# nyenyu12/BioInformatics-project-for-Shotgun-Metagenomics-Pseudo-alignment-shotgun-

Hardware: AMD Instinct MI355X
Metric: reads/sec pseudo-aligned (k=31, 150bp) at 1/2/4/8 GPUs; % HBM roofline (higher is better)
Workload: dtype u8

## Files before the change

bioinformatics-project-for-shotgun-metagenomics-pseudo-alignment-shotgun-_amd/csrc/pa_align.hip:

```cpp
#include <hip/hip_runtime.h>

#include <algorithm>
#include <cstdio>
#include <cstdlib>
#include <cstring>
#include <vector>

#include "pa_device.h"
#include "pa_internal.h"

using namespace pad;

namespace {

constexpr int kBlock = 256;
constexpr int kWaves = kBlock / 64;
constexpr uint32_t kSegMaxWaves = 16384;
constexpr uint32_t kSegSlackWaves = 8192, kSegSlackChunks = 5;
constexpr uint64_t kSegSlack = 64ull * kSegSlackChunks * kSegSlackWaves;
constexpr uint32_t kLdsGenomeCap = 2048;

enum : uint32_t { F_MRQ = 1, F_MKQ = 2, F_MG = 4 };

struct AlignArgs {
// ... 626 lines not shown
                x.type_out[r] = type;
                x.qf_out[r] = qf;
                x.hr_out[r] = hr;
                x.len_out[r] = list_len;
            } else {
                atomicAdd(&a.stats[type == PA_UNMAPPED ? 2 : (type == PA_UNIQUELY_MAPPED ? 0 : 1)], 1ull);
                if (has_mkq && qf) atomicAdd(&a.stats[4], (unsigned long long)qf);
                if (has_mg && hr) atomicAdd(&a.stats[5], (unsigned long long)hr);
            }
        }
        __syncthreads();
    }
}


size_t fast_lds_bytes(uint32_t G, int wpl, bool need_q) {
    size_t cnt = G <= kLdsGenomeCap ? (((size_t)((G + 1) & ~1u) * 16 + 15) / 16 * 16) : 0;
    size_t wl = wpl == 1 ? fast_wave_bytes<1>(need_q) : wpl == 2 ? fast_wave_bytes<2>(need_q) : fast_wave_bytes<4>(need_q);
    return cnt + kWaves * wl;
}

template <int NW, int WPL, bool DENSE>
pa_status launch_fast(const AlignArgs &a, size_t shm, hipStream_t st) {
    auto kern = k_align_fast<NW, WPL, DENSE>;
    if (shm > 64 * 1024) PA_HIP(hipFuncSetAttribute((const void *)kern, hipFuncAttributeMaxDynamicSharedMemorySize, (int)shm));
    int per_cu = 0;
    PA_HIP(hipOccupancyMaxActiveBlocksPerMultiprocessor(&per_cu, kern, kBlock, shm));
    int dev = 0, cus = 256;
    PA_HIP(hipGetDevice(&dev));
    PA_HIP(hipDeviceGetAttribute(&cus, hipDeviceAttributeMultiprocessorCount, dev));
    uint64_t want = (a.n + kWaves - 1) / kWaves;
    uint64_t resident = (uint64_t)std::max(1, per_cu) * (uint64_t)cus;
    unsigned grid = (unsigned)std::max<uint64_t>(1, std::min<uint64_t>(want, resident));
    hipLaunchKernelGGL(kern, dim3(grid), dim3(kBlock), shm, st, a);
    PA_HIP(hipGetLastError());
    return PA_OK;
}

struct KernelTimer {
    pa_index *idx;
    hipStream_t st;
    int slot;
    hipEvent_t e0 = nullptr;
    KernelTimer(pa_index *i, hipStream_t s, int sl) : idx(i), st(s), slot(sl) {
        if (idx && idx->profile && hipEventCreate(&e0) == hipSuccess) hipEventRecord(e0, st);
    }
    ~KernelTimer() {
        hipEvent_t e1 = nullptr;
        if (e0 && hipEventCreate(&e1) == hipSuccess && hipEventRecord(e1, st) == hipSuccess)
            idx->kev.push_back({slot, e0, e1});
        else if (e0)
            hipEventDestroy(e0);
    }
};

constexpr uint64_t kRcnbMinReads = 32768;
pa_status launch_lane(const AlignArgs &a0, hipStream_t st, pa_index *prof = nullptr, bool long_reads = false,
                      int nw = 1) {
    const bool need_q = (a0.prm.flags & (F_MRQ | F_MKQ)) != 0;
    const bool win_q = (a0.prm.flags & F_MKQ) != 0;
    const bool mg = (a0.prm.flags & F_MG) != 0;
    const bool nm4 = long_reads && !win_q && nw == 1;
    AlignArgs a = a0;
    const size_t shm = lane_lds_bytes(a.G, nm4 ? 4 : 2, lane_sched(win_q, mg, nm4 ? 4 : 2, nw));
    auto kern = nw == 3
                    ? (win_q ? (mg ? k_align_lane<true, true, true, 2, 3> : k_align_lane<true, true, false, 2, 3>)
// ... 321 lines not shown

pa_status effective_params(const pa_reads *r, const DevParams &p, DevParams &out, hipStream_t st) {
    out = p;
    if (!(p.flags & (F_MRQ | F_MKQ)) || !r->qual || r->n == 0 || std::getenv("PA_NO_QELIDE")) return PA_OK;
    if (r->q_min < 0) PA_TRY(reads_measure(const_cast<pa_reads *>(r), st));
    if ((p.flags & F_MRQ) && r->len_min > 0 && p.mrq <= r->q_min) out.flags &= ~F_MRQ;
    if ((p.flags & F_MKQ) && p.mkq <= r->q_min) out.flags &= ~F_MKQ;
    return PA_OK;
}

pa_status align(pa_index *idx, const pa_reads *r, const DevParams &p_in, uint64_t base, pa_result *acc,
                hipStream_t st) {
    if (r->n == 0) return PA_OK;
    if (r->n >= 0xFFFFFFFFull) {
        set_error("pa_align: a batch holds at most 2^32 - 2 reads (split it; read_index_base keeps the order)");
        return PA_EUNSUPPORTED;
    }
    PA_TRY(index_note_reads(idx, r->n, st));
    PA_TRY(reserve_queues(idx, r->n));
    DevParams p;
    PA_TRY(effective_params(r, p_in, p, st));
    AlignArgs a = make_args(idx, r, p, base);
    const uint32_t G = idx->n_genomes;
    a.stats = (unsigned long long *)acc->sum_block;
    a.uniq = (unsigned long long *)acc->sum_block + 6;
    a.amb = a.uniq + G;
    a.first = (unsigned long long *)acc->min_block;
    a.queue = idx->queue;
    a.qcount = (unsigned long long *)idx->counters;
    a.deferred_total = (unsigned long long *)idx->counters + 1;
    a.dbg = (unsigned long long *)idx->counters + 4;
    PA_HIP(hipMemsetAsync(idx->counters, 0, 8, st));
#ifdef PA_STATS
    PA_HIP(hipMemsetAsync(a.dbg, 0, 224, st));
#endif
    ExactArgs x{};
    unsigned egrid = 0;
    PA_TRY(prepare_exact(idx, r, x, egrid));
    x.a = a;
    x.detail = 0;
    const bool fast_ok = idx->k > 0 && idx->nw <= 4 && idx->n_kmers > 0;
    const char *no_lane = std::getenv("PA_NO_LANE");
    const bool lane_ok = fast_ok && idx->nw <= 3 && a.tile_n > 0 && a.tile_lw && !(no_lane && no_lane[0] == '1');
    if (fast_ok) {
        const uint32_t wmax = r->max_len >= idx->k ? (uint32_t)(r->max_len - idx->k + 1) : 0;
        const int wpl = wmax <= 64 ? 1 : wmax <= 128 ? 2 : 4;
        hipEvent_t e0 = nullptr, e1 = nullptr;
        if (idx->profile) {
            PA_HIP(hipEventCreate(&e0));
            PA_HIP(hipEventCreate(&e1));
            PA_HIP(hipEventRecord(e0, st));
        }
        if (lane_ok) {
            if ((a.prm.flags & F_MG) && a.prm.mg >= 2) {
                const uint64_t n_words = a.tile_n / 64 + 8;
                if (!idx->tile_big) PA_HIP(pa::dev_malloc(&idx->tile_big, n_words * 8));
                if (idx->tile_big_mg != a.prm.mg) {
                    hipLaunchKernelGGL(k_tile_big, dim3((unsigned)std::min<uint64_t>((n_words + 3) / 4, 1u << 20)),
                                       dim3(256), 0, st, idx->tile_cls, a.tile_n, a.G, idx->class_genomes,
                                       (int32_t)a.prm.mg, idx->tile_big, n_words);
                    PA_HIP(hipGetLastError());
                    idx->tile_big_mg = a.prm.mg;
                }
                a.tile_big = idx->tile_big;
                if (idx->tile_nb && idx->nb_spec && !idx->tile_nb1 && !std::getenv("PA_NO_NBBIG")) {
                    const uint64_t nw = 3 * a.tile_n;
                    if (!idx->tile_nbbig) {
// ... 74 lines not shown
            a.na_min = 32768;
            if (const char *e = std::getenv("PA_NA_MIN")) a.na_min = std::strtoull(e, nullptr, 10);
            a.lane_next = (uint32_t *)(idx->na_count + 3);
            if (na || PA_LANE_CLAIM) PA_HIP(hipMemsetAsync(idx->na_count, 0, 32, st));
            const bool long_reads = r->max_len > (uint32_t)kLaneMaxLen ||
                                    (r->max_len >= idx->k && r->max_len - idx->k + 1 > (uint32_t)kLaneMaxW);
            PA_TRY(launch_lane(a, st, idx, long_reads, idx->nw));
            a.rlist = idx->queue_hard;
            a.rlist_count = a.queue_hard_count;
        }
        {
            KernelTimer kt(idx, st, PA_PROF_WAVE);
            PA_TRY(idx->nw == 1   ? launch_fast_wpl<1>(a, wpl, st)
                   : idx->nw == 2 ? launch_fast_wpl<2>(a, wpl, st)
                   : idx->nw == 3 ? launch_fast_wpl<3>(a, wpl, st)
                                  : launch_fast_wpl<4>(a, wpl, st));
        }
        if (idx->profile) {
            PA_HIP(hipEventRecord(e1, st));
            idx->ev_start.push_back(e0);
            idx->ev_stop.push_back(e1);
        }
        x.a = a;
        x.use_queue = 1;
    } else {
        x.use_queue = 0;
    }
    {
        KernelTimer kt(idx, st, PA_PROF_EXACT);
        launch_exact_nw(idx->nw, x, egrid, st);
        PA_HIP(hipGetLastError());
    }
#ifdef PA_STATS
    unsigned long long d[32];
    PA_HIP(hipMemcpyAsync(d, idx->counters, 256, hipMemcpyDeviceToHost, st));
    PA_HIP(hipStreamSynchronize(st));
    fprintf(stderr, "[pa_stats] reads %llu lane-hard %llu exact %llu | wave kernel: windows %llu probed %llu walk %llu anchors %llu\n",
            (unsigned long long)r->n, d[3], d[0], d[4], d[5], d[6], d[7]);
    fprintf(stderr, "[pa_stats] lane hard reasons: long %llu mkq %llu bad %llu no-anchor %llu range %llu mismatches %llu rep %llu found %llu pending %llu\n",
            d[8], d[9], d[10], d[11], d[12], d[13], d[14], d[15], d[16]);
    fprintf(stderr, "[pa_stats] lane: cooperative probes %llu re-anchors %llu neighbour words %llu | pending: invalid %llu "
            "2+ mismatches %llu neighbour present %llu\n", d[18], d[19], d[20], d[21], d[22], d[23]);
    fprintf(stderr, "[pa_stats] lane found: shared-neighbour+specific %llu second-walk specific %llu probed-shared+specific %llu"
            " | unique by bound %llu, by off-walk counts %llu | probes past the Bloom filter %llu\n", d[24], d[25], d[26], d[27], d[28],
            d[29]);
    fprintf(stderr, "[pa_stats] lane seeds: anchor ranked among stretches %llu, second seed round %llu\n", d[30], d[31]);
#endif
    return PA_OK;
}

pa_status align_detail(pa_index *idx, const pa_reads *r, const DevParams &p, uint8_t *type, uint32_t *qf,
                       uint32_t *hr, uint64_t *list_off, uint32_t *lists, uint64_t list_cap, uint64_t *list_total,
                       hipStream_t st) {
    const uint64_t n = r->n;
    if (list_off) list_off[0] = 0;
    if (list_total) *list_total = 0;
    if (n == 0) return PA_OK;
    ExactArgs x{};
    unsigned egrid = 0;
    PA_TRY(prepare_exact(idx, r, x, egrid));
    x.a = make_args(idx, r, p, 0);
    x.use_queue = 0;
    uint8_t *d_type = nullptr;
    uint32_t *d_qf = nullptr, *d_hr = nullptr, *d_len = nullptr, *d_lists = nullptr;
    uint64_t *d_off = nullptr;
    PA_HIP(pa::dev_malloc(&d_type, n));
    PA_HIP(pa::dev_malloc(&d_qf, n * 4));
    PA_HIP(pa::dev_malloc(&d_hr, n * 4));
    PA_HIP(pa::dev_malloc(&d_len, n * 4));
    x.type_out = d_type;
    x.qf_out = d_qf;
    x.hr_out = d_hr;
    x.len_out = d_len;
    x.detail = 1;
    launch_exact_nw(idx->nw, x, egrid, st);
// ... 65 lines not shown
```

bioinformatics-project-for-shotgun-metagenomics-pseudo-alignment-shotgun-_amd/csrc/pa_fast.h:

```cpp

#ifndef PA_HS_PER_WPL
#define PA_HS_PER_WPL 128
#endif
template <int WPL>
struct FastCfg {
    static constexpr int HS = PA_HS_PER_WPL * WPL;
    static constexpr int E = HS / 64;
    static constexpr int LCAP = 64 * WPL + 64;
    static constexpr int NDW = (LCAP + 8 + 255) / 256;
    static constexpr int PW = NDW * 8 + 2;
    static constexpr int BW = NDW * 4 + 2;
};

template <int WPL>
struct __align__(16) WaveLds {
    using C = FastCfg<WPL>;
    uint64_t packed[C::PW];
    uint64_t diff[C::PW];
    uint64_t poison[C::BW];
    uint64_t hA_key[C::HS];
    uint32_t hA_v[C::HS];
    uint32_t hA_v2[C::HS];
    uint32_t hB_key[C::HS];
    uint32_t hB_cnt[C::HS];
    uint32_t hB_min[C::HS];
    uint32_t gcnt[64];
    uint32_t gmin[64];
};

template <int WPL>
struct __align__(16) WaveQual {
    using C = FastCfg<WPL>;
    uint32_t stage[C::NDW * 64];
// ... 193 lines not shown
        }
#pragma unroll
        for (int e = 0; e < C::E; e++)
            if (bit(specm, e)) count_genome(a, wc, L.hB_key[lane + 64 * e], false, 1, first_key(read_idx, rank[e]));
        return OUT_AMB;
    }
    if (a.prm.p < 0 || nmulti == 0) {
        if (lane == 0) count_genome(a, wc, gstar, true, 1, first_key(read_idx, 0));
        return OUT_UNIQUE;
    }
    wave_sync();
#pragma unroll
    for (int e = 0; e < C::E; e++) {
        const int i = lane + 64 * e;
        L.hA_key[i] = EMPTY;
        L.hA_v[i] = 0;
        L.hA_v2[i] = NONE;
    }
    wave_sync();
    uint32_t ovf = 0;
    const uint32_t limit = (C::HS * 3) / 4;
#pragma unroll
    for (int e = 0; e < C::E; e++)
        if (bit(specm, e)) {
            const int i = lane + 64 * e;
            const uint32_t p = lds_insert64_bounded(L.hA_key, C::HS, L.hB_key[i]);
            if (p >= (uint32_t)C::HS) {
                ovf = 1;
            } else {
                atomicAdd(&L.hA_v[p], L.hB_cnt[i]);
                atomicMin(&L.hA_v2[p], L.hB_min[i]);
            }
        }
#pragma unroll
    for (int f = 0; f < C::E; f++) {
        for (uint64_t m = __ballot(bit(multim, f)); m; m &= m - 1) {
            const uint32_t i = __builtin_ctzll(m) + 64 * f;
            const uint32_t c = L.hB_key[i], cnt = L.hB_cnt[i], mw = L.hB_min[i];
            const uint32_t *rec = a.class_genomes + (c - G);
            const uint32_t sz = rec[0];
            if (sz > limit) {
                ovf = 1;
                break;
            }
            for (uint32_t j = lane; j < sz; j += 64) {
                const uint32_t p = lds_insert64_bounded(L.hA_key, C::HS, rec[1 + j]);
                if (p >= (uint32_t)C::HS) {
                    ovf = 1;
                } else {
                    atomicAdd(&L.hA_v[p], cnt);
                    atomicMin(&L.hA_v2[p], mw);
                }
            }
        }
    }
    wave_sync();
    uint32_t claimed = 0;
#pragma unroll
    for (int e = 0; e < C::E; e++) claimed += (uint32_t)__popcll(__ballot(L.hA_key[lane + 64 * e] != EMPTY));
    if (__ballot(ovf) || claimed > limit) {
        if (lane == 0) a.queue[atomicAdd(a.qcount, 1ull)] = (uint32_t)r;
        return OUT_DEFER;
    }
    uint32_t ts_l = 0, mx_l = 0;
#pragma unroll
    for (int e = 0; e < C::E; e++) {
        const int i = lane + 64 * e;
        if (L.hA_key[i] == EMPTY) continue;
        mx_l = max(mx_l, L.hA_v[i]);
        if (L.hA_key[i] == gstar) ts_l = L.hA_v[i];
    }
    const uint32_t tstar = wave_max(ts_l), maxtot = wave_max(mx_l);
    if ((int64_t)maxtot - (int64_t)tstar > a.prm.p) {
        uint32_t qm = 0;
        uint64_t me[C::E];
        uint32_t rank[C::E];
#pragma unroll
        for (int e = 0; e < C::E; e++) {
            const int i = lane + 64 * e;
            qm |= (L.hA_key[i] != EMPTY && L.hA_v[i] >= tstar ? 1u : 0u) << e;
            me[e] = ((uint64_t)L.hA_v2[i] << 32) | (uint32_t)L.hA_key[i];
            rank[e] = 1;
        }
#pragma unroll
        for (int f = 0; f < C::E; f++) {
            for (uint64_t m = __ballot(bit(qm, f)); m; m &= m - 1) {
                const uint32_t i = __builtin_ctzll(m) + 64 * f;
                const uint64_t other = ((uint64_t)L.hA_v2[i] << 32) | (uint32_t)L.hA_key[i];
// ... 537 lines not shown
    {
        const uint32_t s0 = wave_sum(tot.d_win), s1 = wave_sum(tot.d_probe), s2 = wave_sum(tot.d_walk),
                       s3 = wave_sum(tot.d_anchor);
        if (lane == 0) {
            atomicAdd(&a.dbg[0], (unsigned long long)s0);
            atomicAdd(&a.dbg[1], (unsigned long long)s1);
            atomicAdd(&a.dbg[2], (unsigned long long)s2);
            atomicAdd(&a.dbg[3], (unsigned long long)s3);
        }
    }
#endif
    if (lane == 0) {
        if (tot.unique) atomicAdd(&a.stats[0], (unsigned long long)tot.unique);
        if (tot.mapped > tot.unique) atomicAdd(&a.stats[1], (unsigned long long)(tot.mapped - tot.unique));
        if (tot.unm) atomicAdd(&a.stats[2], (unsigned long long)tot.unm);
        if (tot.drop) atomicAdd(&a.stats[3], (unsigned long long)tot.drop);
        if (qf_w && has_mkq) atomicAdd(&a.stats[4], (unsigned long long)qf_w);
        if (hr_w && has_mg) atomicAdd(&a.stats[5], (unsigned long long)hr_w);
    }
    if (wc.lds) {
        __syncthreads();
        for (uint32_t g = threadIdx.x; g < G; g += kBlock) {
            if (wc.uniq[g]) atomicAdd(&a.uniq[g], (unsigned long long)wc.uniq[g]);
            if (wc.amb[g]) atomicAdd(&a.amb[g], (unsigned long long)wc.amb[g]);
            if (wc.first[g] != (unsigned long long)PA_NO_FIRST_KEY) atomicMin(&a.first[g], wc.first[g]);
        }
    }
}

template <int WPL>
constexpr size_t fast_wave_bytes(bool need_q) {
    return sizeof(WaveLds<WPL>) + (need_q ? sizeof(WaveQual<WPL>) : 0);
}
```

bioinformatics-project-for-shotgun-metagenomics-pseudo-alignment-shotgun-_amd/csrc/pa_index.hip:

```cpp
#include <hip/hip_runtime.h>

#include <algorithm>
#include <cmath>
#include <cstdlib>
#include <cstring>
#include <chrono>
#include <memory>
#include <cstdio>
#include <string>
#include <vector>

#include "pa_device.h"
#include "pa_internal.h"

using namespace pad;

namespace {

constexpr int kBlock = 256;
constexpr int kRun = 16;
#ifndef PA_BATCHED_INSERT
#define PA_BATCHED_INSERT 1
#endif
constexpr bool kBatchedInsert = PA_BATCHED_INSERT != 0;
// ... 2134 lines not shown
            region_goff.assign(n + 1, 0);
            for (uint32_t g = 0; g < n; g++) region_goff[g + 1] = region_goff[g] + strand_region(idx->h_fwd_len[g]);
            goff = region_goff.data();
        }
    }
    idx->h_goff.assign(goff, goff + n + 1);
    const uint64_t total = goff[n] - goff[0];
    uint64_t windows = 0;
    for (uint32_t g = 0; g < n; g++) {
        uint64_t len = goff[g + 1] - goff[g];
        if (both) {
            len = idx->h_fwd_len[g];
            if (k > 0 && (uint64_t)k <= len) windows += 2 * (len - (uint64_t)k + 1);
            continue;
        }
        if (k > 0 && (uint64_t)k <= len) windows += len - (uint64_t)k + 1;
    }
    for (auto &o : idx->h_goff) o -= goff[0];
    idx->total_windows = windows;
    const char *no_tile = std::getenv("PA_NO_TILE");
    uint64_t max_glen = 0;
    for (uint32_t g = 0; g < n; g++) max_glen = std::max<uint64_t>(max_glen, goff[g + 1] - goff[g]);
    idx->tile_n = (idx->nw <= 3 && k > 0 && total > 0 && max_glen < 0xFFFFFFFFull && !(no_tile && no_tile[0] == '1'))
                      ? total : 0;
    idx->tpos_local = total >= 0xFFFFFFFFull ? 1 : 0;
    if (const char *e = std::getenv("PA_LAYOUT")) idx->force_large = std::strcmp(e, "large") == 0;
    if (const char *e = std::getenv("PA_TPOS_LOCAL")) idx->tpos_local |= e[0] == '1';
    idx->tpos_local |= idx->force_large;
    if (dev_codes)
        idx->codes = dev_codes;
    else
        PA_HIP(pa::dev_malloc(&idx->codes, std::max<uint64_t>(total, 1)));
    PA_HIP(pa::dev_malloc(&idx->goff, (n + 1) * 8));
    PA_HIP(pa::dev_malloc(&idx->counters, 32 * 8));
    PA_HIP(hipMemsetAsync(idx->counters, 0, 32 * 8, st));
    PA_HIP(hipMemcpyAsync(idx->goff, idx->h_goff.data(), (n + 1) * 8, hipMemcpyHostToDevice, st));
    if (both) {
        PA_HIP(pa::dev_malloc(&idx->fwd_len, std::max<uint64_t>(n, 1) * 8));
        PA_HIP(hipMemcpyAsync(idx->fwd_len, idx->h_fwd_len.data(), (uint64_t)n * 8, hipMemcpyHostToDevice, st));
    }
    if (total > 0 && !dev_codes && both) {
        uint8_t *ascii = nullptr;
        uint64_t *d_fgoff = nullptr;
        unsigned long long *bad = nullptr, h_bad = ~0ull;
        PA_HIP(pa::dev_malloc(&ascii, fwd_total + kExpandPad));
        PA_HIP(pa::dev_malloc(&d_fgoff, (n + 1) * 8));
        PA_HIP(pa::dev_malloc(&bad, 8));
        tm.mark("alloc");
        hipError_t e = hipMemsetAsync(bad, 0xFF, 8, st);
        if (e == hipSuccess) e = hipMemcpyAsync(d_fgoff, fwd_goff.data(), (n + 1) * 8, hipMemcpyHostToDevice, st);
        if (e == hipSuccess) e = hipMemcpyAsync(ascii, genomes + text_off, fwd_total, hipMemcpyHostToDevice, st);
        tm.mark("upload");
        if (e == hipSuccess) {
            const unsigned grid = grid_for((total + kExpandRun - 1) / kExpandRun);
            hipLaunchKernelGGL(k_encode_strands, dim3(grid > 65536 ? 65536 : grid), dim3(kBlock), 0, st, ascii, d_fgoff,
                               idx->goff, n, idx->codes, bad);
            e = hipMemcpyAsync(&h_bad, bad, 8, hipMemcpyDeviceToHost, st);
        }
        if (e == hipSuccess) e = hipStreamSynchronize(st);
        pa::dev_free(ascii);
        pa::dev_free(d_fgoff);
        pa::dev_free(bad);
        PA_HIP(e);
        if (h_bad != ~0ull) {
            set_error("genome text may only contain A, C, G, T and N (byte " + std::to_string(h_bad) + ")");
            return PA_EINVAL;
        }
    } else if (total > 0 && !dev_codes) {
// ... 350 lines not shown
```

bioinformatics-project-for-shotgun-metagenomics-pseudo-alignment-shotgun-_amd/csrc/pa_lane.h:

```cpp

constexpr uint64_t kPosMask = (1ull << 40) - 1;
template <int NM>
struct LaneShape {
    static constexpr int MAXW = 64 * NM;
    static constexpr int NWD = NM == 2 ? 6 : 9;
    static constexpr int MAXLEN = 32 * NWD - 16;
    static constexpr int NB = NM + 1;
};
constexpr int kLaneMaxW = LaneShape<2>::MAXW;
constexpr int kLaneMaxLen = LaneShape<2>::MAXLEN;
constexpr int kLaneWords = LaneShape<2>::NWD;
#ifndef PA_LANE_MAXMIS
#define PA_LANE_MAXMIS 40
#endif
constexpr uint32_t kLaneMaxMis = PA_LANE_MAXMIS;
#ifndef PA_LANE_PROBES
#define PA_LANE_PROBES 4
#endif
#ifndef PA_LANE_SEEDS
#define PA_LANE_SEEDS 5
#endif
#ifndef PA_SEED_SLOTS
#define PA_SEED_SLOTS 2
#endif
#ifndef PA_LANE_RANK_WORDS
#define PA_LANE_RANK_WORDS 6
#endif
#ifndef PA_LANE_SLOTS
#define PA_LANE_SLOTS 1
#endif
constexpr int kPassEntries = 64 * PA_LANE_PROBES;
#ifndef PA_TWO_WINQ
#define PA_TWO_WINQ 1
#endif
#ifndef PA_LANE_CLAIM
#define PA_LANE_CLAIM 1
#endif
#ifndef PA_LANE_PREOFF
#define PA_LANE_PREOFF 1
#endif
#ifndef PA_LANE_RUN
#define PA_LANE_RUN 2
#endif
constexpr uint32_t kLaneClaimHeld = PA_LANE_CLAIM ? 2 + PA_LANE_RUN : 0;
#ifndef PA_LANE_TOPWAIT
#define PA_LANE_TOPWAIT 1
#endif
#ifndef PA_LANE_LATE
#define PA_LANE_LATE 1
#endif
constexpr int kLaneWaitVm0 = 0x0F70;
constexpr bool lane_sched(bool win_q, bool mg, int nm, int nw) {
    return (PA_LANE_CLAIM || PA_LANE_PREOFF) && nm == 2 && (nw > 1 || !mg);
}
constexpr size_t kLaneOffsBytes = 66 * 8;
#ifndef PA_LANE_LDS_GENOMES
#define PA_LANE_LDS_GENOMES 1664
#endif
constexpr uint32_t lane_lds_genome_cap(bool sched) {
    return sched && PA_LANE_PREOFF ? PA_LANE_LDS_GENOMES - 264 : PA_LANE_LDS_GENOMES;
}

template <int NM>
struct __align__(16) LaneWave {
    uint64_t R[64][LaneShape<NM>::NWD + 1];
    unsigned long long cand[64];
    uint32_t flags[64];
    uint32_t hr[64];
    uint32_t gsp[64];
    uint16_t list[kPassEntries];
    uint32_t again_r[128];
    unsigned long long again_a[128];
};

enum : int {
    LANE_UNIQUE = 0, LANE_AMB = 1, LANE_UNMAPPED = 2, LANE_DROP = 3, LANE_HARD = 4, LANE_WALK = 5, LANE_AGAIN = 6,
    LANE_NOANCHOR = 7
};

template <int N>
__device__ __forceinline__ uint64_t word_at(const uint64_t (&v)[N], uint32_t q) {
    uint64_t r = 0;
#pragma unroll
// ... 693 lines not shown
template <int NM>
__device__ __forceinline__ uint32_t lane_popc(const uint64_t (&m)[NM]) {
    uint32_t x = 0;
#pragma unroll
    for (int i = 0; i < NM; i++) x += (uint32_t)__popcll(m[i]);
    return x;
}

template <int NM>
__device__ __forceinline__ void range_mask(int32_t lo, int32_t hi, uint64_t (&r)[NM]) {
#pragma unroll
    for (int i = 0; i < NM; i++) {
        const int32_t b = 64 * i, l = lo - b, h = hi - b;
        r[i] = (h < 0 || l > 63) ? 0ull
                                 : ((l <= 0 ? ~0ull : (~0ull << l)) & (h >= 63 ? ~0ull : ((2ull << h) - 1)));
    }
}

template <int NM>
__device__ __forceinline__ void or_at(uint64_t (&m)[NM], uint64_t v, int32_t sft) {
#pragma unroll
    for (int i = 0; i < NM; i++) {
        const int32_t s = sft - 64 * i;
        m[i] |= (s >= 64 || s <= -32) ? 0ull : (s >= 0 ? v << s : v >> (-s));
    }
}

template <int NM>
__device__ __forceinline__ void shifted_planes(const uint64_t (&p)[NM + 1], uint32_t fr, uint64_t (&out)[NM]) {
#pragma unroll
    for (int i = 0; i < NM; i++) out[i] = fr ? (p[i] >> fr) | (p[i + 1] << (64 - fr)) : p[i];
}

template <bool WIN_Q, bool MG, int NW = 1>
__device__ __forceinline__ void lane_walk_150(const AlignArgs &a, const uint64_t *row, LaneRead<2> &S) {
    const int k = a.k;
    uint32_t W = S.W, len = S.len;
    asm volatile("" : "+v"(W), "+v"(len));
    const uint64_t atp = S.anc & kPosMask;
    const int64_t A = (int64_t)atp - (int64_t)(S.anc >> 40);
    const bool in_tile = A >= 0 && (uint64_t)A + W <= a.tile_n;
    const uint64_t Ac = in_tile ? (uint64_t)A : 0;
    const uint32_t gr = (uint32_t)(2 * Ac & 63);
    uint64_t gw[kLaneWords + 1], pa3[3], pb3[3];
    lane_blocks<true>(a, Ac, len, gw, pa3, pb3);
    const uint32_t g = S.acls < a.G ? S.acls : genome_of(a.goff, a.gblk, atp);
    S.g = g;
    const uint64_t gs = a.goff[g], ge = a.goff[g + 1];
    if (!in_tile || A < (int64_t)gs || (uint64_t)A + W - 1 + k > ge) {
        S.kind = LANE_HARD;
        return (void)LANE_HARD_WHY(4);
    }
    const uint32_t fr = (uint32_t)(Ac & 63);
    const uint64_t PA0 = fr ? (pa3[0] >> fr) | (pa3[1] << (64 - fr)) : pa3[0];
    const uint64_t PA1 = fr ? (pa3[1] >> fr) | (pa3[2] << (64 - fr)) : pa3[1];
    const uint64_t PB0 = fr ? (pb3[0] >> fr) | (pb3[1] << (64 - fr)) : pb3[0];
    const uint64_t PB1 = fr ? (pb3[1] >> fr) | (pb3[2] << (64 - fr)) : pb3[1];
    const uint64_t IX0 = PA0 | PB0, IX1 = PA1 | PB1;
    uint64_t U0 = 0, U1 = 0, V0 = 0, V1 = 0, NP0 = 0, NP1 = 0, NS0 = 0, NS1 = 0, NG0 = 0, NG1 = 0;
    uint32_t nmis = 0;
    const bool has_nb = a.tile_nb != nullptr;
    uint64_t epk = 0;
    uint32_t cpk = 0;
    uint32_t nnb = 0;
    const uint32_t qlast = (len - 1) >> 5, rl = len - 32 * qlast;
    const uint64_t tail = rl >= 32 ? ~0ull : ~0ull << (64 - 2 * rl);
    auto mismatch = [&](uint32_t e, auto &&sub) -> bool {
// ... 157 lines not shown
            atomicAdd(&a.dbg[16], 1ull);
#endif
            if (sft >= 0) {
                NP0 |= sft < 64 ? nbw << sft : 0ull;
                NP1 |= sft >= 64 ? nbw << (sft - 64) : (sft > 32 ? nbw >> (64 - sft) : 0ull);
                NS0 |= sft < 64 ? nbs << sft : 0ull;
                NS1 |= sft >= 64 ? nbs << (sft - 64) : (sft > 32 ? nbs >> (64 - sft) : 0ull);
                NG0 |= sft < 64 ? nbg << sft : 0ull;
                NG1 |= sft >= 64 ? nbg << (sft - 64) : (sft > 32 ? nbg >> (64 - sft) : 0ull);
            } else {
                NP0 |= nbw >> (-sft);
                NS0 |= nbs >> (-sft);
                NG0 |= nbg >> (-sft);
            }
        }
    }
    if (!has_nb) {
        NP0 = NS0 = ~0ull;
        NP1 = NS1 = ~0ull;
    }
    const bool has_mg = MG;
    const int32_t mgv = a.prm.mg;
    const bool mgk = has_mg && a.mg_nb;
    const uint64_t NB0 = !mgk ? 0ull : (mgv <= 0 ? NP0 : (mgv == 1 ? NP0 & ~NS0 : NG0));
    const uint64_t NB1 = !mgk ? 0ull : (mgv <= 0 ? NP1 : (mgv == 1 ? NP1 & ~NS1 : NG1));
    const uint64_t NQ0 = !has_mg ? NS0 : (mgk ? NS0 & ~NB0 : NP0), NQ1 = !has_mg ? NS1 : (mgk ? NS1 & ~NB1 : NP1);
    const uint64_t in0 = W >= 64 ? ~0ull : ((1ull << W) - 1);
    const uint64_t in1 = W <= 64 ? 0ull : (W >= 128 ? ~0ull : ((1ull << (W - 64)) - 1));
    const uint64_t live0 = WIN_Q ? in0 & ~S.F[0] : in0, live1 = WIN_Q ? in1 & ~S.F[1] : in1;
    const uint64_t valid0 = IX0 & live0, valid1 = IX1 & live1;
    const uint64_t P0 = (live0 & ~valid0) | (valid0 & U0 & (V0 | NQ0));
    const uint64_t P1 = (live1 & ~valid1) | (valid1 & U1 & (V1 | NQ1));
    S.uoff = (uint32_t)(__popcll(valid0 & U0 & ~V0 & NP0 & ~NQ0 & ~NB0) + __popcll(valid1 & U1 & ~V1 & NP1 & ~NQ1 & ~NB1));
    const uint32_t hr_off = (uint32_t)(__popcll(valid0 & U0 & ~V0 & NB0) + __popcll(valid1 & U1 & ~V1 & NB1));
    const uint64_t walked0 = valid0 & ~U0, walked1 = valid1 & ~U1;
#ifdef PA_STATS
    atomicAdd(&a.dbg[17], (unsigned long long)(__popcll(live0 & ~valid0) + __popcll(live1 & ~valid1)));
    atomicAdd(&a.dbg[18], (unsigned long long)(__popcll(valid0 & U0 & V0) + __popcll(valid1 & U1 & V1)));
    atomicAdd(&a.dbg[19], (unsigned long long)(__popcll(valid0 & U0 & NQ0 & ~V0) + __popcll(valid1 & U1 & NQ1 & ~V1)));
#endif
    if ((walked0 & PB0 & ~PA0) | (walked1 & PB1 & ~PA1)) {
        S.kind = LANE_HARD;
        return (void)LANE_HARD_WHY(6);
    }
    const uint64_t spec0 = PA0 & PB0, spec1 = PA1 & PB1;
    uint64_t big0 = 0, big1 = 0;
    if (has_mg) {
        const int32_t mg = a.prm.mg;
        if (mg < 1) {
            big0 = walked0;
            big1 = walked1;
        } else if (mg == 1) {
            big0 = walked0 & ~spec0;
            big1 = walked1 & ~spec1;
        } else {
            const uint64_t *bp = a.tile_big + (Ac >> 6);
            const uint64_t b0 = bp[0], b1 = bp[1], b2 = bp[2];
            big0 = walked0 & ~spec0 & (fr ? (b0 >> fr) | (b1 << (64 - fr)) : b0);
            big1 = walked1 & ~spec1 & (fr ? (b1 >> fr) | (b2 << (64 - fr)) : b1);
        }
    }
    const uint64_t incl0 = walked0 & ~big0, incl1 = walked1 & ~big1;
    const uint32_t hr = (uint32_t)(__popcll(big0) + __popcll(big1));
    const uint32_t nincl = (uint32_t)(__popcll(incl0) + __popcll(incl1));
    const uint32_t nspec = (uint32_t)(__popcll(incl0 & spec0) + __popcll(incl1 & spec1));
    S.nspec = nspec;
    S.nincl = nincl;
    S.hr = hr + hr_off;
    S.P[0] = P0;
    S.P[1] = P1;
    if ((uint32_t)(__popcll(P0) + __popcll(P1)) > a.lane_maxpend) {
        S.kind = LANE_HARD;
        return (void)LANE_HARD_WHY(8);
    }
}

#ifndef PA_LANE_HALVES
#define PA_LANE_HALVES 1
#endif
template <bool MG>
__device__ __forceinline__ void lane_walk_halves(const AlignArgs &a, const uint64_t *row, LaneRead<4> &S) {
    const int64_t A = (int64_t)(S.anc & kPosMask) - (int64_t)(S.anc >> 40);
    const uint32_t len = S.len, W = S.W;
    S.nspec = S.nincl = S.hr = S.uoff = 0;
    S.P[2] = S.P[3] = 0;
#pragma unroll 1
    for (uint32_t h = 0; h < 2; h++) {
        LaneRead<2> H;
        H.kind = LANE_WALK;
        H.F[0] = H.F[1] = 0;
        if (h == 0) {
            H.len = W > 128 ? 127 + (uint32_t)a.k : len;
            H.W = W > 128 ? 128u : W;
            H.anc = S.anc;
            H.acls = S.acls;
        } else {
            H.len = len - 128;
            H.W = W - 128;
            H.anc = (uint64_t)(A + 128);
            H.acls = S.g;
        }
        lane_walk_150<false, MG, 1>(a, row + 4 * h, H);
        if (h == 0) S.g = H.g;
        S.kind = H.kind;
        S.nspec += H.nspec, S.nincl += H.nincl, S.hr += H.hr, S.uoff += H.uoff;
        if (h == 0) {
            S.P[0] = H.P[0], S.P[1] = H.P[1];
        } else {
            S.P[2] = H.P[0], S.P[3] = H.P[1];
        }
        if (S.kind != LANE_WALK || W <= 128) break;
    }
}

template <int NM, bool WIN_Q, bool MG>
__device__ __forceinline__ void lane_walk_long(const AlignArgs &a, const uint64_t *row, LaneRead<NM> &S) {
    using SH = LaneShape<NM>;
    constexpr int NWD = SH::NWD;
    const int k = a.k;
    const uint32_t W = S.W, len = S.len;
    const uint64_t atp = S.anc & kPosMask;
    const int64_t A = (int64_t)atp - (int64_t)(S.anc >> 40);
    const bool in_tile = A >= 0 && (uint64_t)A + W <= a.tile_n;
    const uint64_t Ac = in_tile ? (uint64_t)A : 0;
    const uint32_t gr = (uint32_t)(2 * Ac & 63);
    uint64_t gw[NWD + 1], pa3[NM + 1], pb3[NM + 1];
    lane_blocks<true, NWD, NM + 1>(a, Ac, len, gw, pa3, pb3);
    const uint32_t g = S.acls < a.G ? S.acls : genome_of(a.goff, a.gblk, atp);
    S.g = g;
    const uint64_t gs = a.goff[g], ge = a.goff[g + 1];
    if (!in_tile || A < (int64_t)gs || (uint64_t)A + W - 1 + k > ge) {
        S.kind = LANE_HARD;
        return (void)LANE_HARD_WHY(4);
    }
    const uint32_t fr = (uint32_t)(Ac & 63);
    uint64_t PA[NM], PB[NM];
    shifted_planes<NM>(pa3, fr, PA);
    shifted_planes<NM>(pb3, fr, PB);
    uint64_t U[NM], V[NM], NP[NM], NS[NM], NG[NM];
#pragma unroll
    for (int i = 0; i < NM; i++) U[i] = V[i] = NP[i] = NS[i] = NG[i] = 0;
    uint32_t nmis = 0;
    const bool has_nb = a.tile_nb != nullptr;
    uint64_t epk = 0;
// ... 277 lines not shown
                                                                               a.goff, a.tpos_local));
            }
        }
        wave_sync();
    }
}

#ifndef PA_LANE_WAVES
#define PA_LANE_WAVES 4
#endif

#ifndef PA_LANE_WAVES_Q
#define PA_LANE_WAVES_Q 4
#endif
#ifndef PA_LANE_WAVES_LONG
#define PA_LANE_WAVES_LONG 4
#endif
#ifndef PA_LANE_WAVES_MG
#define PA_LANE_WAVES_MG 4
#endif
#ifndef PA_LANE_WAVES_W
#define PA_LANE_WAVES_W 3
#endif
template <bool NEED_Q, bool WIN_Q, bool MG, int NM = 2, int NW = 1>
__global__ __launch_bounds__(kBlock) __attribute__((amdgpu_waves_per_eu(
    NM == 4 ? PA_LANE_WAVES_LONG
            : (NW >= 2 ? PA_LANE_WAVES_W : (WIN_Q ? PA_LANE_WAVES_Q : (MG ? PA_LANE_WAVES_MG : PA_LANE_WAVES))))))
void k_align_lane(AlignArgs a) {
    using LW_t = LaneWave<NM>;
    constexpr int NWD = LaneShape<NM>::NWD;
    extern __shared__ __align__(16) unsigned char smem[];
    const uint32_t G = a.G;
    const int lane = lane_id();
    constexpr bool kSched = lane_sched(WIN_Q, MG, NM, NW);
    const bool lds = G <= lane_lds_genome_cap(kSched);
    const size_t cnt_bytes = lds ? ((size_t)G * 8 + 15) / 16 * 16 : 0;
    uint32_t *first = (uint32_t *)smem;
    uint32_t *uniq = first + (lds ? G : 0);
    LW_t &LW = ((LW_t *)(smem + cnt_bytes))[__builtin_amdgcn_readfirstlane(threadIdx.x >> 6)];
    uint64_t *noff = nullptr;
    if constexpr (kSched && PA_LANE_PREOFF)
        noff = (uint64_t *)(smem + cnt_bytes + kWaves * sizeof(LW_t) +
                            kLaneOffsBytes * (uint32_t)__builtin_amdgcn_readfirstlane(threadIdx.x >> 6));
    if (lds) {
        for (uint32_t i = threadIdx.x; i < G; i += kBlock) {
            first[i] = ~0u;
            uniq[i] = 0;
        }
        __syncthreads();
    }
    uint32_t n_uniq = 0, n_amb = 0, n_unm = 0, n_drop = 0;
    uint64_t n_hr = 0, n_qf = 0;
    LW.R[lane][NWD] = 0;
    constexpr bool CLAIM = PA_LANE_CLAIM && kSched, PREOFF = PA_LANE_PREOFF && kSched;
    const uint64_t n_chunks = (a.n + 63) / 64, wave_stride = (uint64_t)gridDim.x * kWaves;
    uint64_t chunk = (uint64_t)blockIdx.x * kWaves + (uint32_t)__builtin_amdgcn_readfirstlane(threadIdx.x >> 6);
    uint64_t chunk1 = chunk + wave_stride;
    auto chunk_offs = [&](uint64_t c, uint64_t &o0, uint64_t &o1) {
        const uint64_t i = c * 64 + (uint32_t)lane;
        o1 = a.off[i + 1 < a.n ? i + 1 : a.n];
        if (lane == 0) o0 = a.off[i];
    };
    if constexpr (PREOFF) {
        if (chunk < n_chunks) {
            uint64_t o0 = 0, o1;
            chunk_offs(chunk, o0, o1);
            noff[lane + 1] = o1;
// ... 87 lines not shown
                    if (nres) {
                        chunk1 = res++;
                        nres--;
                    } else if (claimed) {
                        chunk1 = 2 * wave_stride + (uint32_t)__builtin_amdgcn_readfirstlane(cl);
                        res = chunk1 + 1;
                        nres = run - 1;
                    } else {
                        chunk1 = ~0ull;
                    }
                } else
                    chunk1 += wave_stride;
            }
            if (packed) lane_seeds<NM, NW>(a, cd, my_row(), S);
        }
#if defined(PA_STATS) || defined(PA_DISSECT)
        if (a.dbg_mode == 10 && S.kind == LANE_WALK) S.kind = LANE_AMB;
#endif
#pragma unroll 1
        for (int attempt = again_batch ? 1 : 0; attempt < 2; attempt++) {
            if (S.kind == LANE_WALK) {
                if constexpr (NM == 2)
                    lane_walk_150<WIN_Q, MG, NW>(a, my_row(), S);
                else
                    if constexpr (NM == 4 && !WIN_Q && NW == 1 && PA_LANE_HALVES)
                        lane_walk_halves<MG>(a, my_row(), S);
                    else
                        lane_walk_long<NM, WIN_Q, MG>(a, my_row(), S);
            }
#if defined(PA_STATS) || defined(PA_DISSECT)
            if (a.dbg_mode == 11 && S.kind == LANE_WALK) S.kind = LANE_AMB;
#endif
            if (!__ballot(S.kind == LANE_WALK)) break;
            if (S.kind == LANE_WALK && S.nspec > 0 && (!MG || (a.mg_nb && !lane_any(S.P)))) {
                const int64_t X = (int64_t)(lane_popc(S.P) + S.uoff);
                const int64_t ns = (int64_t)S.nspec;
                if (ns >= X + (a.prm.m > 0 ? a.prm.m : 1) && (a.prm.p < 0 || X - ns <= a.prm.p)) {
                    S.kind = LANE_UNIQUE;
#ifdef PA_STATS
                    atomicAdd(&a.dbg[23], 1ull);
#endif
                }
            }
            if (S.kind == LANE_WALK && S.uoff && S.nspec > 0 && MG && !a.mg_nb) {
                S.kind = LANE_HARD;
                LANE_HARD_WHY(7);
                LANE_HARD_WHY(16);
            }
            lane_probe_wave<NM, NW, PA_TWO_WINQ || !WIN_Q>(a, LW, S, S.P, true);
            if (S.kind == LANE_WALK) {
                const uint32_t fl = LW.flags[lane];
                const uint32_t nsoff = fl >> 16;
                bool two = false;
                if ((PA_TWO_WINQ || !WIN_Q) && (!MG || a.mg_nb) && nsoff && !(fl & 2u) && LW.gsp[lane] != S.g + 1) {
                    const int64_t ns = (int64_t)S.nspec, c = (int64_t)nsoff;
                    const int64_t noff = (int64_t)(((fl >> 2) & 0x3FFFu) + S.uoff);
                    two = ns >= c + (a.prm.m > 0 ? a.prm.m : 1) && (a.prm.p < 0 || noff + c - ns <= a.prm.p);
                }
                if (two) {
                    S.kind = LANE_UNIQUE;
                    if (MG) S.hr += LW.hr[lane];
#ifdef PA_STATS
                    atomicAdd(&a.dbg[24], 1ull);
#endif
                } else if (nsoff) {
#if defined(PA_STATS) || defined(PA_DISSECT)
                    if (a.dbg_mode == 12) S.kind = LANE_AMB;
#endif
                    if (S.kind != LANE_WALK) {
                    } else if (attempt == 0) {
#ifdef PA_STATS
                        atomicAdd(&a.dbg[15], 1ull);
#endif
                        S.kind = LANE_AGAIN;
                    } else {
                        S.kind = LANE_HARD;
                        LANE_HARD_WHY(7);
                        LANE_HARD_WHY(17);
                    }
                } else {
                    if (MG) S.hr += LW.hr[lane];
                    const uint32_t noff = ((fl >> 2) & 0x3FFFu) + S.uoff;
                    if (noff) {
// ... 779 lines not shown
```

Before: 4.354 billion.

## Flatten multi-genome class expansion into a wave-wide prefix-scanned work list

Replaces the serial per-class loop, where each multi-genome class is expanded across lanes one at a time, with a flattened scheme. Class offsets and sizes are prefix-scanned and compacted into LDS, and each lane binary-searches its global work index, so small classes no longer leave most lanes idle. Count and min are packed into 16-bit halves, which assumes both fit in 16 bits. It also adds an environment override to cap the fast-kernel grid size, plus a static_assert on the LDS budget.

```diff
diff --git a/bioinformatics-project-for-shotgun-metagenomics-pseudo-alignment-shotgun-_amd/csrc/pa_align.hip b/bioinformatics-project-for-shotgun-metagenomics-pseudo-alignment-shotgun-_amd/csrc/pa_align.hip
--- a/bioinformatics-project-for-shotgun-metagenomics-pseudo-alignment-shotgun-_amd/csrc/pa_align.hip
+++ b/bioinformatics-project-for-shotgun-metagenomics-pseudo-alignment-shotgun-_amd/csrc/pa_align.hip
@@ -682,6 +682,8 @@
     uint64_t want = (a.n + kWaves - 1) / kWaves;
     uint64_t resident = (uint64_t)std::max(1, per_cu) * (uint64_t)cus;
     unsigned grid = (unsigned)std::max<uint64_t>(1, std::min<uint64_t>(want, resident));
+    if (const char *e = std::getenv("PA_FAST_GRID"))
+        grid = (unsigned)std::max<uint64_t>(1, std::min<uint64_t>(grid, std::strtoull(e, nullptr, 10)));
     hipLaunchKernelGGL(kern, dim3(grid), dim3(kBlock), shm, st, a);
     PA_HIP(hipGetLastError());
     return PA_OK;
diff --git a/bioinformatics-project-for-shotgun-metagenomics-pseudo-alignment-shotgun-_amd/csrc/pa_fast.h b/bioinformatics-project-for-shotgun-metagenomics-pseudo-alignment-shotgun-_amd/csrc/pa_fast.h
--- a/bioinformatics-project-for-shotgun-metagenomics-pseudo-alignment-shotgun-_amd/csrc/pa_fast.h
+++ b/bioinformatics-project-for-shotgun-metagenomics-pseudo-alignment-shotgun-_amd/csrc/pa_fast.h
@@ -1,4 +1,7 @@
 
+#ifndef PA_FAST_SETS
+#define PA_FAST_SETS 1
+#endif
 #ifndef PA_HS_PER_WPL
 #define PA_HS_PER_WPL 128
 #endif
@@ -258,6 +261,78 @@
                 atomicMin(&L.hA_v2[p], L.hB_min[i]);
             }
         }
+#if PA_FAST_SETS
+    {
+        uint32_t ro[C::E], sz[C::E], cm[C::E];
+        uint32_t big = 0;
+#pragma unroll
+        for (int e = 0; e < C::E; e++) {
+            const int i = lane + 64 * e;
+            ro[e] = sz[e] = cm[e] = 0;
+            if (bit(multim, e)) {
+                ro[e] = L.hB_key[i] - G;
+                cm[e] = (L.hB_cnt[i] << 16) | L.hB_min[i];
+                sz[e] = a.class_genomes[ro[e]];
+            }
+        }
+#pragma unroll
+        for (int e = 0; e < C::E; e++) big |= sz[e] > limit ? 1u : 0u;
+        if (__ballot(big)) {
+            ovf = 1;
+        } else {
+            wave_sync();
+            uint32_t nset = 0, total = 0;
+#pragma unroll
+            for (int e = 0; e < C::E; e++) {
+                const uint64_t b = __ballot(bit(multim, e));
+                const uint32_t inc = wave_incl_scan(sz[e]);
+                if (bit(multim, e)) {
+                    const uint32_t at = nset + lanes_below(b);
+                    L.hB_key[at] = ro[e];
+                    L.hB_cnt[at] = cm[e];
+                    L.hB_min[at] = total + inc;
+                }
+                nset += (uint32_t)__popcll(b);
+                total += (uint32_t)__builtin_amdgcn_readlane(inc, 63);
+            }
+            wave_sync();
+            constexpr int kSetSteps = 2;
+            for (uint32_t t0 = 0; t0 < total; t0 += 64 * kSetSteps) {
+                uint32_t g[kSetSteps], v[kSetSteps];
+#pragma unroll
+                for (int u = 0; u < kSetSteps; u++) {
+                    const uint32_t t = t0 + 64 * u + lane;
+                    g[u] = NONE;
+                    v[u] = 0;
+                    if (t < total) {
+                        uint32_t lo = 0, hi = nset - 1;
+                        while (lo < hi) {
+                            const uint32_t mid = (lo + hi) >> 1;
+                            if (L.hB_min[mid] > t)
+                                hi = mid;
+                            else
+                                lo = mid + 1;
+                        }
+                        const uint32_t start = lo ? L.hB_min[lo - 1] : 0u;
+                        g[u] = a.class_genomes[L.hB_key[lo] + 1 + (t - start)];
+                        v[u] = L.hB_cnt[lo];
+                    }
+                }
+#pragma unroll
+                for (int u = 0; u < kSetSteps; u++)
+                    if (t0 + 64 * u + lane < total) {
+                        const uint32_t p = lds_insert64_bounded(L.hA_key, C::HS, g[u]);
+                        if (p >= (uint32_t)C::HS) {
+                            ovf = 1;
+                        } else {
+                            atomicAdd(&L.hA_v[p], v[u] >> 16);
+                            atomicMin(&L.hA_v2[p], v[u] & 0xFFFFu);
+                        }
+                    }
+            }
+        }
+    }
+#else
 #pragma unroll
     for (int f = 0; f < C::E; f++) {
         for (uint64_t m = __ballot(bit(multim, f)); m; m &= m - 1) {
@@ -280,6 +355,7 @@
             }
         }
     }
+#endif
     wave_sync();
     uint32_t claimed = 0;
 #pragma unroll
@@ -883,3 +959,4 @@
 constexpr size_t fast_wave_bytes(bool need_q) {
     return sizeof(WaveLds<WPL>) + (need_q ? sizeof(WaveQual<WPL>) : 0);
 }
+static_assert(kWaves * sizeof(WaveLds<2>) + 16 * 500 <= 160 * 1024 / 4, "WaveLds<2>: four blocks per CU at 500 genomes");
```

Result: no change. 4.389 billion, median of 6 (+0.8%).

## Short-circuit lane walk with a single sure re-anchor probe when ambiguity is certain

Applied to the files above, without the earlier changes.

Adds a 'sure' path in the 150bp and long lane walks. When enough specific-but-off k-mers are found that the read cannot be resolved as unique, the walk keeps only one pending window, the first such candidate, and marks it with a flag bit. The probe stage then either re-anchors from that window (LANE_AGAIN) or sends the read to the hard/exact path. This is meant to avoid probing many pending windows and running the two-neighbour analysis. In exchange more reads may take a second walk or fall to the exact kernel. The counter arrays grow to hold the extra stats.

```diff
diff --git a/bioinformatics-project-for-shotgun-metagenomics-pseudo-alignment-shotgun-_amd/csrc/pa_align.hip b/bioinformatics-project-for-shotgun-metagenomics-pseudo-alignment-shotgun-_amd/csrc/pa_align.hip
--- a/bioinformatics-project-for-shotgun-metagenomics-pseudo-alignment-shotgun-_amd/csrc/pa_align.hip
+++ b/bioinformatics-project-for-shotgun-metagenomics-pseudo-alignment-shotgun-_amd/csrc/pa_align.hip
@@ -1069,7 +1069,7 @@
     a.dbg = (unsigned long long *)idx->counters + 4;
     PA_HIP(hipMemsetAsync(idx->counters, 0, 8, st));
 #ifdef PA_STATS
-    PA_HIP(hipMemsetAsync(a.dbg, 0, 224, st));
+    PA_HIP(hipMemsetAsync(a.dbg, 0, 36 * 8, st));
 #endif
     ExactArgs x{};
     unsigned egrid = 0;
@@ -1210,8 +1210,8 @@
         PA_HIP(hipGetLastError());
     }
 #ifdef PA_STATS
-    unsigned long long d[32];
-    PA_HIP(hipMemcpyAsync(d, idx->counters, 256, hipMemcpyDeviceToHost, st));
+    unsigned long long d[40];
+    PA_HIP(hipMemcpyAsync(d, idx->counters, sizeof d, hipMemcpyDeviceToHost, st));
     PA_HIP(hipStreamSynchronize(st));
     fprintf(stderr, "[pa_stats] reads %llu lane-hard %llu exact %llu | wave kernel: windows %llu probed %llu walk %llu anchors %llu\n",
             (unsigned long long)r->n, d[3], d[0], d[4], d[5], d[6], d[7]);
@@ -1219,6 +1219,7 @@
             d[8], d[9], d[10], d[11], d[12], d[13], d[14], d[15], d[16]);
     fprintf(stderr, "[pa_stats] lane: cooperative probes %llu re-anchors %llu neighbour words %llu | pending: invalid %llu "
             "2+ mismatches %llu neighbour present %llu\n", d[18], d[19], d[20], d[21], d[22], d[23]);
+    fprintf(stderr, "[pa_stats] lane: single-probe re-anchors %llu second walks given up unprobed %llu\n", d[32], d[33]);
     fprintf(stderr, "[pa_stats] lane found: shared-neighbour+specific %llu second-walk specific %llu probed-shared+specific %llu"
             " | unique by bound %llu, by off-walk counts %llu | probes past the Bloom filter %llu\n", d[24], d[25], d[26], d[27], d[28],
             d[29]);
diff --git a/bioinformatics-project-for-shotgun-metagenomics-pseudo-alignment-shotgun-_amd/csrc/pa_index.hip b/bioinformatics-project-for-shotgun-metagenomics-pseudo-alignment-shotgun-_amd/csrc/pa_index.hip
--- a/bioinformatics-project-for-shotgun-metagenomics-pseudo-alignment-shotgun-_amd/csrc/pa_index.hip
+++ b/bioinformatics-project-for-shotgun-metagenomics-pseudo-alignment-shotgun-_amd/csrc/pa_index.hip
@@ -2190,8 +2190,8 @@
     else
         PA_HIP(pa::dev_malloc(&idx->codes, std::max<uint64_t>(total, 1)));
     PA_HIP(pa::dev_malloc(&idx->goff, (n + 1) * 8));
-    PA_HIP(pa::dev_malloc(&idx->counters, 32 * 8));
-    PA_HIP(hipMemsetAsync(idx->counters, 0, 32 * 8, st));
+    PA_HIP(pa::dev_malloc(&idx->counters, 40 * 8));
+    PA_HIP(hipMemsetAsync(idx->counters, 0, 40 * 8, st));
     PA_HIP(hipMemcpyAsync(idx->goff, idx->h_goff.data(), (n + 1) * 8, hipMemcpyHostToDevice, st));
     if (both) {
         PA_HIP(pa::dev_malloc(&idx->fwd_len, std::max<uint64_t>(n, 1) * 8));
diff --git a/bioinformatics-project-for-shotgun-metagenomics-pseudo-alignment-shotgun-_amd/csrc/pa_lane.h b/bioinformatics-project-for-shotgun-metagenomics-pseudo-alignment-shotgun-_amd/csrc/pa_lane.h
--- a/bioinformatics-project-for-shotgun-metagenomics-pseudo-alignment-shotgun-_amd/csrc/pa_lane.h
+++ b/bioinformatics-project-for-shotgun-metagenomics-pseudo-alignment-shotgun-_amd/csrc/pa_lane.h
@@ -49,6 +49,13 @@
 #ifndef PA_LANE_LATE
 #define PA_LANE_LATE 1
 #endif
+#ifndef PA_LANE_SURE
+#define PA_LANE_SURE 1
+#endif
+constexpr uint32_t kLaneSure = 1u << 31;
+constexpr bool lane_sure(bool win_q, bool mg, int nm, int nw) {
+    return PA_LANE_SURE && nw == 1 && (nm == 2 || !mg);
+}
 constexpr int kLaneWaitVm0 = 0x0F70;
 constexpr bool lane_sched(bool win_q, bool mg, int nm, int nw) {
     return (PA_LANE_CLAIM || PA_LANE_PREOFF) && nm == 2 && (nw > 1 || !mg);
@@ -808,7 +815,7 @@
     for (int i = 0; i < NM; i++) out[i] = fr ? (p[i] >> fr) | (p[i + 1] << (64 - fr)) : p[i];
 }
 
-template <bool WIN_Q, bool MG, int NW = 1>
+template <bool WIN_Q, bool MG, int NW = 1, int SURE = lane_sure(WIN_Q, MG, 2, NW)>
 __device__ __forceinline__ void lane_walk_150(const AlignArgs &a, const uint64_t *row, LaneRead<2> &S) {
     const int k = a.k;
     uint32_t W = S.W, len = S.len;
@@ -1032,6 +1039,14 @@
     const uint64_t P0 = (live0 & ~valid0) | (valid0 & U0 & (V0 | NQ0));
     const uint64_t P1 = (live1 & ~valid1) | (valid1 & U1 & (V1 | NQ1));
     S.uoff = (uint32_t)(__popcll(valid0 & U0 & ~V0 & NP0 & ~NQ0 & ~NB0) + __popcll(valid1 & U1 & ~V1 & NP1 & ~NQ1 & ~NB1));
+    uint32_t sure = 0;
+    if constexpr (SURE != 0 && NW == 1) {
+        if (has_nb && a.nb_spec && (!has_mg || mgk)) {
+            const uint64_t C0 = valid0 & U0 & ~V0 & NQ0, C1 = valid1 & U1 & ~V1 & NQ1;
+            sure = (uint32_t)(__popcll(C0) + __popcll(C1)) |
+                   ((C0 ? (uint32_t)__builtin_ctzll(C0) : 64u + (uint32_t)__builtin_ctzll(C1 | (1ull << 63))) << 8);
+        }
+    }
     const uint32_t hr_off = (uint32_t)(__popcll(valid0 & U0 & ~V0 & NB0) + __popcll(valid1 & U1 & ~V1 & NB1));
     const uint64_t walked0 = valid0 & ~U0, walked1 = valid1 & ~U1;
 #ifdef PA_STATS
@@ -1069,6 +1084,18 @@
     S.hr = hr + hr_off;
     S.P[0] = P0;
     S.P[1] = P1;
+    if constexpr (SURE == 2) {
+        S.uoff |= sure << 8;
+    } else if constexpr (SURE == 1 && NW == 1) {
+        const uint32_t cs = sure & 255u;
+        if (cs && nspec < cs + (uint32_t)(a.prm.m > 0 ? a.prm.m : 1)) {
+            const uint32_t w = sure >> 8;
+            S.P[0] = w < 64 ? 1ull << w : 0ull;
+            S.P[1] = w < 64 ? 0ull : 1ull << (w - 64);
+            S.uoff = kLaneSure;
+            return;
+        }
+    }
     if ((uint32_t)(__popcll(P0) + __popcll(P1)) > a.lane_maxpend) {
         S.kind = LANE_HARD;
         return (void)LANE_HARD_WHY(8);
@@ -1084,6 +1111,7 @@
     const uint32_t len = S.len, W = S.W;
     S.nspec = S.nincl = S.hr = S.uoff = 0;
     S.P[2] = S.P[3] = 0;
+    uint32_t cs = 0, sw = 0;
 #pragma unroll 1
     for (uint32_t h = 0; h < 2; h++) {
         LaneRead<2> H;
@@ -1100,16 +1128,25 @@
             H.anc = (uint64_t)(A + 128);
             H.acls = S.g;
         }
-        lane_walk_150<false, MG, 1>(a, row + 4 * h, H);
+        lane_walk_150<false, MG, 1, lane_sure(false, MG, 4, 1) ? 2 : 0>(a, row + 4 * h, H);
         if (h == 0) S.g = H.g;
         S.kind = H.kind;
-        S.nspec += H.nspec, S.nincl += H.nincl, S.hr += H.hr, S.uoff += H.uoff;
+        S.nspec += H.nspec, S.nincl += H.nincl, S.hr += H.hr, S.uoff += H.uoff & 255u;
+        if (H.kind == LANE_WALK && (H.uoff & 0xFF00u)) {
+            if (!cs) sw = 128 * h + ((H.uoff >> 16) & 255u);
+            cs += (H.uoff >> 8) & 255u;
+        }
         if (h == 0) {
             S.P[0] = H.P[0], S.P[1] = H.P[1];
         } else {
             S.P[2] = H.P[0], S.P[3] = H.P[1];
         }
         if (S.kind != LANE_WALK || W <= 128) break;
+    }
+    if (S.kind == LANE_WALK && cs && S.nspec < cs + (uint32_t)(a.prm.m > 0 ? a.prm.m : 1)) {
+#pragma unroll
+        for (uint32_t q = 0; q < 4; q++) S.P[q] = (sw >> 6) == q ? 1ull << (sw & 63) : 0ull;
+        S.uoff = kLaneSure;
     }
 }
 
@@ -1453,7 +1490,7 @@
     extern __shared__ __align__(16) unsigned char smem[];
     const uint32_t G = a.G;
     const int lane = lane_id();
-    constexpr bool kSched = lane_sched(WIN_Q, MG, NM, NW);
+    constexpr bool kSched = lane_sched(WIN_Q, MG, NM, NW), kSure = lane_sure(WIN_Q, MG, NM, NW);
     const bool lds = G <= lane_lds_genome_cap(kSched);
     const size_t cnt_bytes = lds ? ((size_t)G * 8 + 15) / 16 * 16 : 0;
     uint32_t *first = (uint32_t *)smem;
@@ -1607,7 +1644,16 @@
             if (a.dbg_mode == 11 && S.kind == LANE_WALK) S.kind = LANE_AMB;
 #endif
             if (!__ballot(S.kind == LANE_WALK)) break;
-            if (S.kind == LANE_WALK && S.nspec > 0 && (!MG || (a.mg_nb && !lane_any(S.P)))) {
+            const bool sure = kSure && S.kind == LANE_WALK && (S.uoff & kLaneSure);
+            if (sure && attempt == 1) {
+                S.kind = LANE_HARD;
+                LANE_HARD_WHY(7);
+                LANE_HARD_WHY(17);
+#ifdef PA_STATS
+                atomicAdd(&a.dbg[29], 1ull);
+#endif
+            }
+            if (S.kind == LANE_WALK && !sure && S.nspec > 0 && (!MG || (a.mg_nb && !lane_any(S.P)))) {
                 const int64_t X = (int64_t)(lane_popc(S.P) + S.uoff);
                 const int64_t ns = (int64_t)S.nspec;
                 if (ns >= X + (a.prm.m > 0 ? a.prm.m : 1) && (a.prm.p < 0 || X - ns <= a.prm.p)) {
@@ -1623,7 +1669,21 @@
                 LANE_HARD_WHY(16);
             }
             lane_probe_wave<NM, NW, PA_TWO_WINQ || !WIN_Q>(a, LW, S, S.P, true);
-            if (S.kind == LANE_WALK) {
+            if (kSure && S.kind == LANE_WALK && (S.uoff & kLaneSure)) {
+                if (LW.cand[lane] != ~0ull) {
+                    S.kind = LANE_AGAIN;
+#ifdef PA_STATS
+                    atomicAdd(&a.dbg[15], 1ull);
+                    atomicAdd(&a.dbg[28], 1ull);
+#endif
+                } else {
+                    S.kind = LANE_HARD;
+                    LANE_HARD_WHY(7);
+                }
+#if defined(PA_STATS) || defined(PA_DISSECT)
+                if (a.dbg_mode == 12) S.kind = LANE_AMB;
+#endif
+            } else if (S.kind == LANE_WALK) {
                 const uint32_t fl = LW.flags[lane];
                 const uint32_t nsoff = fl >> 16;
                 bool two = false;
```

New measurement: 4.327 billion before, 4.520 billion after (median of 6 runs). 4.5% higher.
